# VinAIResearch/tise-toolbox

Hardware: AMD Instinct MI355X
Metric: images/sec through InceptionV3+FID on 30k 256x256 @1/2/4/8 GPU; |dFID| vs ref (higher is better)
Workload: dtype f32 (split 2xf16 operands, 3 f16 MFMAs/product, f32 accumulate)

## Files before the change

include/tise_hip.h:

```cpp
#ifndef TISE_HIP_H
#define TISE_HIP_H

#include <stddef.h>
#include <stdint.h>

#ifdef __cplusplus
extern "C" {
#endif

#define TISE_OK 0
#define TISE_ERR_INVALID_ARG (-1)
#define TISE_ERR_HIP (-2)
#define TISE_ERR_NO_DEVICE (-3)
#define TISE_ERR_UNSUPPORTED (-4)

const char* tise_status_string(int status);
int tise_last_hip_error(void);
int tise_version(void);
int tise_device_info(int* cu_count, int* gcn_arch_is_gfx950, size_t* total_mem);

int tise_host_register(void* host_ptr, size_t bytes);
int tise_host_unregister(void* host_ptr);
int tise_memcpy_h2d_async(void* dst_dev, const void* src_host, size_t bytes, void* stream);

// ... 105 lines not shown
                                            void* stream);
int tise_maxpool3s1p1_split_nhwc(const void* x_dev, int64_t x_ld, int x_off, int n, int h, int w,
                                 int C, void* out_dev, int64_t out_ld, int out_off, void* stream);

int tise_stem_conv3x3s2_split(const float* x_dev, int n, int h, int w, const float* w_dev, const float* bias_dev,
                              void* out_dev, void* stream);
int tise_stem_conv3x3s2_split_u8(const uint8_t* x_dev, const float* lut_dev, int n, int h, int w, const float* w_dev,
                                 const float* bias_dev, void* out_dev, void* stream);
int tise_stem_conv3x3s2_split_u8_mfma(const uint8_t* x_dev, const float* lut_dev, int n, int h, int w, const void* wsplit_dev,
                                      const float* scale_dev, const float* bias_dev, void* out_dev, void* stream);
int tise_split_mean_nhwc(const void* x_dev, int n, int hw, int C, float* out_dev, void* stream);
int tise_split_mean_both_nhwc(const void* x_dev, int n, int hw, int C, float* out_dev, void* out_split_dev, void* stream);

int tise_cosine_top1(const void* img_emb_dev, const void* txt_emb_dev, const int32_t* txt_index_dev, int64_t n, int c,
                     int d, int dtype, int normalize, float logit_scale, int32_t* top1_out_dev, float* p0_out_dev,
                     void* stream);

int tise_gemm_f16(const void* a_dev, int64_t lda, const void* w_dev, int64_t ldw, const void* bias_dev, const void* res_dev,
                  int64_t ldr, void* out_dev, int64_t ldo, int m, int n, int k, int act, void* stream);
int tise_layernorm_f16(const void* x_dev, int64_t ldx, const void* gamma_dev, const void* beta_dev, void* out_dev, int64_t ldo,
                       int64_t rows, int C, float eps, void* stream);
int tise_attention_f16(const void* qkv_dev, int batch, int seq, int heads, int head_dim, int causal, void* out_dev, void* stream);
int tise_patchify_f16(const void* img_dev, int batch, int res, int patch, void* out_dev, void* stream);
int tise_vit_tokens_f16(const void* patch_out_dev, const void* class_emb_dev, const void* pos_emb_dev, int batch, int n_patches,
                        int width, void* x_dev, void* stream);
int tise_text_tokens_f16(const int32_t* tokens_dev, const void* table_dev, const void* pos_emb_dev, int64_t rows, int seq, int width,
                         void* x_dev, void* stream);
int tise_gather_rows_f16(const void* x_dev, const int64_t* index_dev, int64_t n, int width, void* out_dev, void* stream);

typedef struct {
    int c0, c1;
    void* dst;
    long long ld;
    int off;
    int mode;
} tise_conv_seg;

typedef struct {
    const void* x;
    const void* w;
    long long w_plane;
    const float* scale;
    const float* bias;
    int N, H, W, Cin, KH, KW, SH, SW, PH, PW, OH, OW;
    int Cout, K, Kpad;
    long long M;
    int nseg;
    tise_conv_seg seg[4];
    int out_hp, out_wp, out_y0, out_x0;
} tise_conv_args;

int tise_conv_split_f16(const tise_conv_args* args, int tn, void* stream);

int tise_split_overflow_check(int* flag_host, void* stream);

int tise_gemm_f64(const double* a_dev, int64_t sam, int64_t sak, const double* b_dev, int64_t sbk,
                  int64_t sbn, double* c_dev, int64_t ldc, int m, int n, int k, void* stream);

#ifdef __cplusplus
}
#endif
#endif
```

tise_toolbox_amd/_lib.py:

```python
import ctypes
import os
from ctypes import POINTER, c_char_p, c_double, c_float, c_int, c_int64, c_size_t, c_uint8, c_void_p

_HERE = os.path.dirname(os.path.abspath(__file__))
LIB_PATH = os.environ.get("TISE_LIB_PATH") or os.path.join(_HERE, "libtise_hip.so")


class TiseLibraryError(RuntimeError):
    pass


class TiseStatusError(RuntimeError):
    def __init__(self, fn, status, detail):
        super().__init__(f"{fn} failed: {detail} (status {status})")
        self.status = status


TISE_OK = 0
TISE_ERR_INVALID_ARG = -1
TISE_ERR_HIP = -2
TISE_ERR_NO_DEVICE = -3
TISE_ERR_UNSUPPORTED = -4
TISE_FRECHET_OUT_DOUBLES = 8
TISE_FLAG_NONFINITE = 1
# ... 41 lines not shown
    "tise_mmd_poly3_workspace_bytes": (c_int, [POINTER(c_int64), POINTER(c_int64), c_int, POINTER(c_size_t)]),
    "tise_mmd_poly3_grouped": (c_int, [c_void_p, c_int64, c_int64, c_void_p, c_int64, POINTER(c_int64), c_void_p, c_int64, c_int64,
                                        c_void_p, c_int64, POINTER(c_int64), c_int, c_int, c_void_p, c_void_p, c_size_t, c_void_p]),
    "tise_mmd_rbf_workspace_bytes": (c_int, [POINTER(c_int64), POINTER(c_int64), c_int, POINTER(c_size_t)]),
    "tise_mmd_rbf_grouped": (c_int, [c_void_p, c_int64, c_int64, c_void_p, c_int64, POINTER(c_int64), c_void_p, c_int64, c_int64,
                                      c_void_p, c_int64, POINTER(c_int64), c_int, c_int, c_double, c_void_p, c_void_p, c_size_t,
                                      c_void_p]),
    "tise_knn_workspace_bytes": (c_int, [c_int64, c_int, c_int, POINTER(c_size_t)]),
    "tise_knn_radius2": (c_int, [c_void_p, c_int64, c_int64, c_int, c_int, c_int, c_void_p, c_void_p, c_size_t, c_void_p]),
    "tise_prdc_counts": (c_int, [c_void_p, c_int64, c_int64, c_void_p, c_void_p, c_int64, c_int64, c_void_p, c_int, c_int, c_void_p,
                                  c_void_p, c_void_p, c_void_p, c_size_t, c_void_p]),
    "tise_frechet_create": (c_int, [c_int, POINTER(c_void_p)]),
    "tise_frechet_destroy": (c_int, [c_void_p]),
    "tise_frechet_distance": (c_int, [c_void_p, c_void_p, c_void_p, c_void_p, c_void_p, c_double, c_void_p, c_void_p]),
    "tise_frechet_prefactor": (c_int, [c_void_p, c_void_p, c_void_p]),
    "tise_frechet_distance_prefactored": (c_int, [c_void_p, c_void_p, c_void_p, c_void_p, c_void_p, c_void_p, c_void_p]),
    "tise_frechet_prefactor_ms": (c_int, [c_void_p, POINTER(c_double)]),
    "tise_frechet_set_profiling": (c_int, [c_void_p, c_int]),
    "tise_frechet_phase_ms": (c_int, [c_void_p, POINTER(c_double), POINTER(c_int)]),
    "tise_eigvalsh": (c_int, [c_void_p, c_void_p, c_int, c_void_p, c_void_p]),
    "tise_pivoted_cholesky": (c_int, [c_void_p, c_void_p, c_void_p, POINTER(c_int), c_void_p]),
    "tise_frechet_factor": (c_int, [c_void_p, c_void_p, POINTER(c_int), POINTER(c_int), c_void_p]),
    "tise_is_update": (c_int, [c_void_p, c_int64, c_int64, c_int, c_double, c_int, c_int64, c_int64, c_int, c_int,
                                c_void_p, c_void_p, c_void_p]),
    "tise_is_finalize": (c_int, [c_void_p, c_int, c_int64, c_int, c_int, c_void_p, c_void_p]),
    "tise_calib_workspace_bytes": (c_int, [c_int64, c_int, c_int, POINTER(c_size_t)]),
    "tise_calib_eval": (c_int, [c_void_p, c_int64, c_int64, c_int, c_int, c_void_p, c_double, c_void_p, c_int, c_void_p,
                                 c_void_p, c_size_t, c_void_p]),
    "tise_bias_relu_nhwc": (c_int, [c_void_p, c_int64, c_int, c_int64, c_int, c_void_p, c_void_p, c_int64, c_int, c_void_p]),
    "tise_avgpool3_bias_relu_nhwc": (c_int, [c_void_p, c_int64, c_int, c_int, c_int, c_int, c_int, c_void_p, c_void_p,
                                              c_int64, c_int, c_void_p]),
    "tise_maxpool3s2_nhwc": (c_int, [c_void_p, c_int64, c_int, c_int, c_int, c_int, c_int, c_void_p, c_void_p, c_int64,
                                      c_int, c_void_p]),
    "tise_avgpool3_bias_relu_split_nhwc": (c_int, [c_void_p, c_int64, c_int, c_int, c_int, c_int, c_int, c_void_p,
                                                    c_void_p, c_int64, c_int, c_void_p]),
    "tise_maxpool3s2_split_nhwc": (c_int, [c_void_p, c_int64, c_int, c_int, c_int, c_int, c_int, c_void_p,
                                            c_int64, c_int, c_void_p]),
    "tise_avgpool3_excl_bias_relu_nhwc": (c_int, [c_void_p, c_int64, c_int, c_int, c_int, c_int, c_int, c_void_p, c_void_p,
                                                   c_int64, c_int, c_void_p]),
    "tise_maxpool3s1p1_nhwc": (c_int, [c_void_p, c_int64, c_int, c_int, c_int, c_int, c_int, c_void_p, c_int64, c_int,
                                        c_void_p]),
    "tise_avgpool3_excl_bias_relu_split_nhwc": (c_int, [c_void_p, c_int64, c_int, c_int, c_int, c_int, c_int, c_void_p,
                                                         c_void_p, c_int64, c_int, c_void_p]),
    "tise_maxpool3s1p1_split_nhwc": (c_int, [c_void_p, c_int64, c_int, c_int, c_int, c_int, c_int, c_void_p,
                                              c_int64, c_int, c_void_p]),
    "tise_stem_conv3x3s2_split": (c_int, [c_void_p, c_int, c_int, c_int, c_void_p, c_void_p, c_void_p, c_void_p]),
    "tise_stem_conv3x3s2_split_u8": (c_int, [c_void_p, c_void_p, c_int, c_int, c_int, c_void_p, c_void_p, c_void_p,
                                              c_void_p]),
    "tise_stem_conv3x3s2_split_u8_mfma": (c_int, [c_void_p, c_void_p, c_int, c_int, c_int, c_void_p, c_void_p, c_void_p,
                                                   c_void_p, c_void_p]),
    "tise_split_mean_nhwc": (c_int, [c_void_p, c_int, c_int, c_int, c_void_p, c_void_p]),
    "tise_split_mean_both_nhwc": (c_int, [c_void_p, c_int, c_int, c_int, c_void_p, c_void_p, c_void_p]),
    "tise_conv_split_f16": (c_int, [c_void_p, c_int, c_void_p]),
    "tise_split_overflow_check": (c_int, [POINTER(c_int), c_void_p]),
    "tise_gemm_f64": (c_int, [c_void_p, c_int64, c_int64, c_void_p, c_int64, c_int64, c_void_p, c_int64,
                               c_int, c_int, c_int, c_void_p]),
}

_lib = None


def load():
    global _lib
    if _lib is not None:
        return _lib
    if not os.path.exists(LIB_PATH):
        raise TiseLibraryError(
            f"{LIB_PATH} not found: build it with `python -m tise_toolbox_amd.build` "
            "(hipcc --offload-arch=gfx950).  There is no CPU fallback.")
    try:
        lib = ctypes.CDLL(LIB_PATH)
    except OSError as e:
        raise TiseLibraryError(f"cannot load {LIB_PATH}: {e}") from e
    for name, (res, args) in SIGNATURES.items():
        try:
            fn = getattr(lib, name)
        except AttributeError as e:
            raise TiseLibraryError(f"{LIB_PATH} does not export {name}") from e
        fn.restype = res
        fn.argtypes = args
    _lib = lib
    return lib


def check(fn_name, status):
    if status != TISE_OK:
        lib = load()
        detail = lib.tise_status_string(status).decode()
        if status == TISE_ERR_HIP:
            detail += f" (hipError_t {lib.tise_last_hip_error()})"
        raise TiseStatusError(fn_name, status, detail)


def call(fn_name, *args):
    lib = load()
    status = getattr(lib, fn_name)(*args)
    check(fn_name, status)
```

tise_toolbox_amd/csrc/conv_split.hip:

```cpp
#include <hip/hip_fp16.h>
#include "common.h"
#include "conv_epilogue.h"

typedef _Float16 half8_t __attribute__((ext_vector_type(8)));
typedef float float16_t __attribute__((ext_vector_type(16)));
typedef float float4_t __attribute__((ext_vector_type(4)));
typedef unsigned int u32x4_t __attribute__((ext_vector_type(4)));

#define CS_BM 128
#define CS_BK 32

typedef tise_conv_seg ConvSeg;
typedef tise_conv_args ConvArgs;

__device__ u32x4_t g_conv_zero_page[4];

typedef __attribute__((address_space(3))) void* lds_ptr_t;

template <int TN>
__global__ __launch_bounds__(256, 2) void conv_split_glds_kernel(const ConvArgs p) {
    constexpr int BN = 32 * TN;
    constexpr int A_PLANE = CS_BM * 64, B_PLANE = BN * 64;
    constexpr int STAGE = 2 * A_PLANE + 2 * B_PLANE;
    constexpr int T_BYTES = CS_BM * (BN * 2 + 16);
// ... 62 lines not shown
        if (a_c >= p.Cin) { a_c -= p.Cin; if (++a_kw == p.KW) { a_kw = 0; ++a_kh; } }                      \
        if (a_c >= p.Cin) { a_c -= p.Cin; if (++a_kw == p.KW) { a_kw = 0; ++a_kh; } }                      \
    }

    conv_epi::Acc16 acc_main[1][TN], acc_corr[1][TN];
#pragma unroll
    for (int t = 0; t < TN; ++t) { conv_epi::acc_zero(acc_main[0][t]); conv_epi::acc_zero(acc_corr[0][t]); }
    conv_epi::float4_t sc_pre = {0.f, 0.f, 0.f, 0.f}, bs_pre = {0.f, 0.f, 0.f, 0.f};
    if (tid < BN / 4) {
        sc_pre = *reinterpret_cast<const conv_epi::float4_t*>(p.scale + n0 + 4 * tid);
        bs_pre = *reinterpret_cast<const conv_epi::float4_t*>(p.bias + n0 + 4 * tid);
    }

    const int nsteps = p.Kpad / CS_BK;
    const int frow = (lane & 15) * 64;
    const int choff = (((lane >> 4)) ^ (((lane & 15) >> 2) & 3)) * 16;
    CG_ISSUE(0, lds)
    for (int step = 0; step < nsteps; ++step) {
        unsigned char* cur = lds + (step & 1) * STAGE;
        asm volatile("s_waitcnt vmcnt(0)" ::: "memory");
        __syncthreads();
        if (step + 1 < nsteps) CG_ISSUE(step + 1, lds + ((step + 1) & 1) * STAGE)
        half8_t a_[2][2];
#pragma unroll
        for (int pi = 0; pi < 2; ++pi) {
            const unsigned char* ap = cur + (wave * 32 + pi * 16) * 64 + frow + choff;
            a_[pi][0] = *reinterpret_cast<const half8_t*>(ap);
            a_[pi][1] = *reinterpret_cast<const half8_t*>(ap + A_PLANE);
        }
#pragma unroll
        for (int g = 0; g < 2 * TN; ++g) {
            const unsigned char* bp = cur + 2 * A_PLANE + g * 16 * 64 + frow + choff;
            const half8_t b_hi = *reinterpret_cast<const half8_t*>(bp);
            const half8_t b_lo = *reinterpret_cast<const half8_t*>(bp + B_PLANE);
#pragma unroll
            for (int pi = 0; pi < 2; ++pi) {
                float4_t& cm = acc_main[0][g >> 1].v[g & 1][pi];
                float4_t& cc = acc_corr[0][g >> 1].v[g & 1][pi];
                cm = __builtin_amdgcn_mfma_f32_16x16x32_f16(b_hi, a_[pi][0], cm, 0, 0, 0);
                cc = __builtin_amdgcn_mfma_f32_16x16x32_f16(b_lo, a_[pi][0], cc, 0, 0, 0);
                cc = __builtin_amdgcn_mfma_f32_16x16x32_f16(b_hi, a_[pi][1], cc, 0, 0, 0);
            }
        }
    }
    __syncthreads();
    constexpr int ETW = TN > 1 ? 2 : 1;
    constexpr int EPI0 = 4 * conv_epi::Staging<ETW>::BYTES;
    static_assert(EPI0 + conv_epi::EpiArea<BN>::BYTES <= LDS_BYTES, "epilogue staging must fit the operand LDS");
    conv_epi::prepare<BN>(p, lds + EPI0, n0, sc_pre, bs_pre);
    __syncthreads();
    conv_epi::store_tiles_desc<TN, ETW>(p, acc_main, acc_corr, lds + wave * conv_epi::Staging<ETW>::BYTES, lds + EPI0, m0 + wave * 32);
}

template <int TN, bool DBG = false, bool CBT = false>
__global__ __launch_bounds__(256, 2) void conv_split_fast_kernel(const ConvArgs p) {
    constexpr int BN = 32 * TN;
    constexpr int A_BYTES = CS_BM * 128, B_BYTES = BN * 128;
    constexpr int STAGE = A_BYTES + B_BYTES;
    constexpr int T_BYTES = CS_BM * (BN * 2 + 16);
    constexpr int LDS_BYTES = (2 * STAGE > T_BYTES) ? 2 * STAGE : T_BYTES;
    __shared__ __attribute__((aligned(1024))) unsigned char lds[LDS_BYTES];

    const int tid = threadIdx.x, lane = tid & 63;
    const int wave = __builtin_amdgcn_readfirstlane(tid >> 6);
    const unsigned tiles_n = (unsigned)(p.Cout + BN - 1) / BN;
    const unsigned nwg = gridDim.x;
    unsigned bid = blockIdx.x;
    {
        const unsigned q = nwg >> 3, r = nwg & 7, xcd = bid & 7, idx = bid >> 3;
        bid = ((xcd < r) ? xcd * (q + 1) : r * (q + 1) + (xcd - r) * q) + idx;
    }
    const unsigned tile_m = bid / tiles_n;
    const int tile_n = (int)(bid - tile_m * tiles_n);
    const long long m0 = (long long)tile_m * CS_BM;
    const int n0 = tile_n * BN;

    const unsigned char* zp = reinterpret_cast<const unsigned char*>(g_conv_zero_page);
    const int pix_bytes = p.Cin * 4;
    const unsigned char* pbase[4];
    int ihw[4];
    {
        const unsigned ohw = (unsigned)(p.OH * p.OW), M32 = (unsigned)p.M;
        const unsigned pix0 = tile_m * CS_BM + wave * 32 + (lane >> 3);
        const unsigned pp = pix0 < M32 ? pix0 : 0u;
        unsigned n = pp / ohw;
        const unsigned rem = pp - n * ohw;
        unsigned oh = rem / (unsigned)p.OW, ow = rem - oh * (unsigned)p.OW;
#pragma unroll
        for (int jj = 0; jj < 4; ++jj) {
            const int ih0 = (int)oh * p.SH - p.PH, iw0 = (int)ow * p.SW - p.PW;
            const bool rok = pix0 + 8 * jj < M32;
            ihw[jj] = rok ? ((ih0 + 0x4000) << 16) | (iw0 + 0x4000) : 0;
            pbase[jj] = reinterpret_cast<const unsigned char*>(p.x) +
                        (((long long)n * p.H + ih0) * p.W + iw0) * pix_bytes;
            ow += 8;
            while (ow >= (unsigned)p.OW) { ow -= (unsigned)p.OW; if (++oh == (unsigned)p.OH) { oh = 0; ++n; } }
        }
    }
    const unsigned char* wbase = reinterpret_cast<const unsigned char*>(p.w) + (long long)n0 * p.Kpad * 4;
    unsigned pb[TN];
    int pb_off[TN];
#pragma unroll
    for (int i = 0; i < TN; ++i) {
        const int q = wave * TN + i;
        const int r = q * 8 + (lane >> 3);
        const int c = (lane & 7) ^ tise_lds_swz(r);
        pb[i] = (unsigned)r * (unsigned)p.Kpad * 4u + c * 16;
        pb_off[i] = A_BYTES + q * 1024;
    }
    const unsigned char* pa[4];
    int pa_inc[4];
    int kh = 0, kw = 0, cblk = 0, istep = 0;
    const int ncblk = p.Cin / CS_BK, ntaps = p.KH * p.KW;
    const int nA = ntaps * ncblk;
    const int nB = (p.Cin & 16) ? (ntaps + 1) / 2 : 0;
    const int cl0 = (lane & 7) ^ ((lane >> 4) << 1), cl1 = cl0;
#define CF_TAP_ONE(JJ, KH_, KW_, CHB_, VALID_)                                                            \
    {                                                                                                     \
        const int ih = (ihw[JJ] >> 16) - 0x4000 + (KH_), iw = (ihw[JJ] & 0xffff) - 0x4000 + (KW_);         \
        const bool ok = (VALID_) && ih >= 0 && ih < p.H && iw >= 0 && iw < p.W;                            \
        const unsigned char* src = pbase[JJ] + ((KH_) * p.W + (KW_)) * pix_bytes + (CHB_);                 \
        pa[JJ] = ok ? src : zp;                                                                            \
        pa_inc[JJ] = ok ? 128 : 0;                                                                         \
    }
#define CF_TAP()                                                                                          \
    _Pragma("unroll") for (int jj = 0; jj < 4; ++jj) CF_TAP_ONE(jj, kh, kw, ((jj & 1) ? cl1 : cl0) * 16, kh < p.KH)
#define CF_TAP_B(J)                                                                                       \
    _Pragma("unroll") for (int par = 0; par < 2; ++par) {                                                  \
        const int c_ = par ? cl1 : cl0;                                                                    \
        const int tl = 2 * (J) + ((c_ >> 1) & 1);                                                          \
        const int lkh = tl / p.KW, lkw = tl - lkh * p.KW;                                                  \
        const int chb = ncblk * 128 + (c_ >> 2) * 32 + (c_ & 1) * 16;                                      \
        CF_TAP_ONE(par, lkh, lkw, chb, tl < ntaps)                                                         \
        CF_TAP_ONE(par + 2, lkh, lkw, chb, tl < ntaps)                                                     \
    }
#define CF_ISSUE(STAGEOFF)                                                                                \
    {                                                                                                     \
        _Pragma("unroll") for (int jj = 0; jj < 4; ++jj) {                                                 \
                                                     \
            const unsigned char* sa = pa[jj];                                                              \
             \
            if (!(DBG && (p.nseg & 0x1000)) || istep % 7 == 0)                                             \
                __builtin_amdgcn_global_load_lds(sa, (lds_ptr_t)(lds + (STAGEOFF) + (4 * wave + jj) * 1024), 16, 0, 0); \
            pa[jj] = sa + pa_inc[jj];                                                                      \
        }                                                                                                  \
        _Pragma("unroll") for (int i = 0; i < TN; ++i) {                                                   \
            const unsigned char* sw_ = wbase + pb[i];                                                      \
            unsigned char* dw_ = lds + (STAGEOFF) + pb_off[i];                                             \
            __builtin_amdgcn_global_load_lds(sw_, (lds_ptr_t)dw_, 16, 0, 0);                               \
            pb[i] += 128;                                              \
        }                                                                                                  \
        ++istep;                                              \
        if constexpr (CBT) {                                  \
            int delta = pix_bytes - 128;                      \
            if (++kw == p.KW) {                                                                            \
                kw = 0;                                                                                    \
                delta = (p.W - p.KW + 1) * pix_bytes - 128;          \
                if (++kh == p.KH) { kh = 0; delta = -((p.KH - 1) * p.W + (p.KW - 1)) * pix_bytes; }    \
            }                                                                                              \
            _Pragma("unroll") for (int jj = 0; jj < 4; ++jj) pa[jj] += (long long)(pa_inc[jj] ? delta : 0); \
        } else if (istep >= nA) {                                                        \
            if (istep < nA + nB) CF_TAP_B(istep - nA)                                                      \
        } else if (++cblk == ncblk) {                                                 \
            cblk = 0;                                                                                      \
            if (++kw == p.KW) { kw = 0; ++kh; }                                                            \
            CF_TAP()                                                                                       \
        }                                                                                                  \
    }

    constexpr bool W22 = TN == 4;
    constexpr int NPH = W22 ? 4 : 2;
    constexpr int NCH = W22 ? TN : 2 * TN;
    constexpr int RG = NPH / 2, TNW = NCH / 2;
    const int wm = W22 ? (wave & 1) : wave, wn = W22 ? (wave >> 1) : 0;
    conv_epi::Acc16 acc_main[RG][1][TNW], acc_corr[RG][1][TNW];
#pragma unroll
    for (int r = 0; r < RG; ++r)
#pragma unroll
        for (int t = 0; t < TNW; ++t) { conv_epi::acc_zero(acc_main[r][0][t]); conv_epi::acc_zero(acc_corr[r][0][t]); }
    constexpr bool PRE = TN < 5;
    conv_epi::float4_t sc_pre = {0.f, 0.f, 0.f, 0.f}, bs_pre = {0.f, 0.f, 0.f, 0.f};
    if (PRE && tid < BN / 4) {
        sc_pre = *reinterpret_cast<const conv_epi::float4_t*>(p.scale + n0 + 4 * tid);
        bs_pre = *reinterpret_cast<const conv_epi::float4_t*>(p.bias + n0 + 4 * tid);
    }

    const int nsteps = nA + nB;
    const int f16o = (lane & 15) * 128 + (((lane >> 4) ^ tise_lds_swz(lane & 15)) << 4);
    const unsigned char* fa = lds + wm * NPH * 2048;
    const int fbw = A_BYTES + wn * NCH * 2048;
    half8_t h_a[NPH][2], h_b[2];

#define CF_HEAD(STAGEOFF)                                                                                 \
    {                                                                                                     \
        _Pragma("unroll") for (int pi = 0; pi < NPH; ++pi) {                                               \
            h_a[pi][0] = *reinterpret_cast<const half8_t*>(fa + (STAGEOFF) + pi * 2048 + f16o);            \
            h_a[pi][1] = *reinterpret_cast<const half8_t*>(fa + (STAGEOFF) + pi * 2048 + (f16o ^ 64));     \
        }                                                                                                  \
        h_b[0] = *reinterpret_cast<const half8_t*>(lds + (STAGEOFF) + fbw + f16o);                         \
        h_b[1] = *reinterpret_cast<const half8_t*>(lds + (STAGEOFF) + fbw + (f16o ^ 64));                  \
        __builtin_amdgcn_sched_barrier(0);                                                                 \
    }
#define CF_COMPUTE(STAGEOFF)                                                                              \
    {                                                                                                     \
        __builtin_amdgcn_sched_barrier(0);                                                                 \
        half8_t fb_[NCH][2];                                                                               \
        _Pragma("unroll") for (int g = 0; g < NCH; ++g) {                                                  \
            if (g == 0) { fb_[0][0] = h_b[0]; fb_[0][1] = h_b[1]; }                                        \
            else {                                                                                         \
                const unsigned char* bb = lds + (STAGEOFF) + fbw + g * 2048;                               \
                fb_[g][0] = *reinterpret_cast<const half8_t*>(bb + f16o);                                  \
                fb_[g][1] = *reinterpret_cast<const half8_t*>(bb + (f16o ^ 64));                           \
            }                                                                                              \
        }                                                                                                  \
        _Pragma("unroll") for (int g = 0; g < NCH; ++g)                                                    \
            _Pragma("unroll") for (int pi = 0; pi < NPH; ++pi) {                                           \
                           \
                float4_t& cm = acc_main[pi >> 1][0][g >> 1].v[g & 1][pi & 1];                              \
                float4_t& cc = acc_corr[pi >> 1][0][g >> 1].v[g & 1][pi & 1];                              \
                cc = __builtin_amdgcn_mfma_f32_16x16x32_f16(fb_[g][1], h_a[pi][0], cc, 0, 0, 0);           \
                cm = __builtin_amdgcn_mfma_f32_16x16x32_f16(fb_[g][0], h_a[pi][0], cm, 0, 0, 0);           \
                cc = __builtin_amdgcn_mfma_f32_16x16x32_f16(fb_[g][0], h_a[pi][1], cc, 0, 0, 0);           \
            }                                                                                              \
        _Pragma("unroll") for (int g = 0; g < NCH; ++g) {                                                  \
            if (g + 1 < NCH) __builtin_amdgcn_sched_group_barrier(0x100, 2, 0);              \
            __builtin_amdgcn_sched_group_barrier(0x008, 3 * NPH, 0);                        \
        }                                                                                                  \
    }

    const bool ab_dma = !(p.nseg & 0x100), ab_mma = !(p.nseg & 0x200);
    const bool dbg = DBG && (p.nseg & 0x800) && blockIdx.x == 0;
    int* dbuf = reinterpret_cast<int*>(p.seg[3].dst);
#define CF_STAMP(STEP, K)                                                                                  \
    if (DBG && dbg && lane == 0 && (STEP) < 96) dbuf[wave * 512 + (STEP) * 5 + (K)] = (int)__builtin_readcyclecounter();
    if (dbg && lane == 0) dbuf[wave * 512 + 480] = (int)(__builtin_amdgcn_s_memrealtime());
#define CF_BAR() { __builtin_amdgcn_sched_barrier(0); __builtin_amdgcn_s_barrier(); __builtin_amdgcn_sched_barrier(0); }
    int step = 0;
    CF_TAP()
    CF_ISSUE(0)
    for (; step + 1 < nsteps; step += 2) {
        CF_STAMP(step, 0)
        asm volatile("s_waitcnt vmcnt(0)" ::: "memory");
        CF_STAMP(step, 1)
        __syncthreads();
        CF_STAMP(step, 2)
        CF_HEAD(0)
        if (ab_dma) CF_ISSUE(STAGE)
        CF_STAMP(step, 3)
        if (ab_mma) CF_COMPUTE(0)
        CF_STAMP(step, 4)
        CF_STAMP(step + 1, 0)
        asm volatile("s_waitcnt vmcnt(0)" ::: "memory");
        CF_STAMP(step + 1, 1)
        __syncthreads();
        CF_STAMP(step + 1, 2)
        CF_HEAD(STAGE)
        if (step + 2 < nsteps && ab_dma) CF_ISSUE(0)
        CF_STAMP(step + 1, 3)
        if (ab_mma) CF_COMPUTE(STAGE)
        CF_STAMP(step + 1, 4)
    }
    if (dbg && lane == 0) dbuf[wave * 512 + 481] = (int)(__builtin_amdgcn_s_memrealtime());
    if (step < nsteps) {
        asm volatile("s_waitcnt vmcnt(0)" ::: "memory");
        __syncthreads();
        CF_HEAD(0)
        CF_COMPUTE(0)
    }
    __syncthreads();
    if ((p.nseg & 0x400) && p.M > 0) return;
    constexpr int ETW = TN > 1 ? 2 : 1;
    constexpr int EPI0 = 4 * conv_epi::Staging<ETW>::BYTES;
    static_assert(EPI0 + conv_epi::EpiArea<BN>::BYTES <= LDS_BYTES, "epilogue staging must fit the operand LDS");
    if (!PRE && tid < BN / 4) {
        sc_pre = *reinterpret_cast<const conv_epi::float4_t*>(p.scale + n0 + 4 * tid);
        bs_pre = *reinterpret_cast<const conv_epi::float4_t*>(p.bias + n0 + 4 * tid);
    }
    conv_epi::prepare<BN>(p, lds + EPI0, n0, sc_pre, bs_pre, tid);
    __syncthreads();
#pragma unroll
    for (int r = 0; r < RG; ++r)
        conv_epi::store_tiles_desc<TNW, ETW, false, BN>(p, acc_main[r], acc_corr[r], lds + wave * conv_epi::Staging<ETW>::BYTES, lds + EPI0,
                                                        m0 + wm * NPH * 16 + r * 32, wn * NCH * 2);
}


template <int TN, int NP, bool POOLH = false>
__global__ __launch_bounds__(256, 2) void conv_split_rowwin_kernel(const ConvArgs p, const unsigned inv_wp) {
    constexpr int BN = 32 * TN;
    constexpr int MSTEP = POOLH ? 126 : CS_BM;
    constexpr int A_BYTES = NP * 4 * 1024;
    constexpr int B_BYTES = BN * 128;
    constexpr int B0 = 2 * A_BYTES;
    constexpr int LDS_BYTES = 2 * A_BYTES + 2 * B_BYTES;
    extern __shared__ __attribute__((aligned(1024))) unsigned char lds[];

    const int tid = threadIdx.x, lane = tid & 63;
    const int wave = __builtin_amdgcn_readfirstlane(tid >> 6);
    const unsigned tiles_n = (unsigned)(p.Cout + BN - 1) / BN;
    const unsigned nwg = gridDim.x;
    unsigned bid = blockIdx.x;
    {
        const unsigned q = nwg >> 3, r = nwg & 7, xcd = bid & 7, idx = bid >> 3;
        bid = ((xcd < r) ? xcd * (q + 1) : r * (q + 1) + (xcd - r) * q) + idx;
    }
    const unsigned tile_m = bid / tiles_n;
    const int tile_n = (int)(bid - tile_m * tiles_n);
    const long long m0 = (long long)tile_m * MSTEP;
    const int n0 = tile_n * BN;
    const unsigned char* zp = reinterpret_cast<const unsigned char*>(g_conv_zero_page);
    const int pix_bytes = p.Cin * 4;
    const int Wp = p.OW + p.KW - 1;
    const unsigned row0 = (unsigned)(tile_m * MSTEP) / (unsigned)p.OW;
    const int x0 = (int)(tile_m * MSTEP - row0 * (unsigned)p.OW);
    const unsigned img0 = row0 / (unsigned)p.OH;
    const int oy0 = (int)(row0 - img0 * (unsigned)p.OH);
    const unsigned nrows_out = (unsigned)p.N * (unsigned)p.OH;

    const unsigned char* pbase[NP];
    int oyp[NP];
    const int cch = (lane & 7) ^ ((lane >> 4) << 1);
    const int full_off = cch * 16;
    const int tail_off = (cch >> 2) * 32 + (cch & 1) * 16;
    const bool tail_has = (cch & 3) < 2;
#pragma unroll
    for (int t = 0; t < NP; ++t) {
        const int q = wave + 4 * t;
        const int rho = 8 * q + (lane >> 3);
        const unsigned u = (unsigned)(rho + x0);
        const unsigned j = (u * inv_wp) >> 16;
        const int xin = (int)(u - j * (unsigned)Wp) - p.PW;
        unsigned n = img0;
        int oy = oy0 + (int)j;
        while (oy >= p.OH) { oy -= p.OH; ++n; }
        const bool okx = xin >= 0 && xin < p.W && row0 + j < nrows_out;
        oyp[t] = okx ? oy - p.PH + 0x4000 : 0;
// ... 371 lines not shown
        __syncthreads();
        if (step + 1 < nsteps) PI_B_ISSUE(((step + 1) & 1) * B_BYTES)
        half8_t a_[2][2];
#pragma unroll
        for (int pi = 0; pi < 2; ++pi) {
            a_[pi][0] = *reinterpret_cast<const half8_t*>(fa + pi * 2048 + f16o);
            a_[pi][1] = *reinterpret_cast<const half8_t*>(fa + pi * 2048 + (f16o ^ 64));
        }
#pragma unroll
        for (int g = 0; g < 2 * TNW; ++g) {
            const unsigned char* bb = lds + A_BYTES + bcur + (wn * 2 * TNW + g) * 2048;
            const half8_t b_hi = *reinterpret_cast<const half8_t*>(bb + f16o);
            const half8_t b_lo = *reinterpret_cast<const half8_t*>(bb + (f16o ^ 64));
#pragma unroll
            for (int pi = 0; pi < 2; ++pi) {
                float4_t& cm = acc_main[0][g >> 1].v[g & 1][pi];
                float4_t& cc = acc_corr[0][g >> 1].v[g & 1][pi];
                cc = __builtin_amdgcn_mfma_f32_16x16x32_f16(b_lo, a_[pi][0], cc, 0, 0, 0);
                cm = __builtin_amdgcn_mfma_f32_16x16x32_f16(b_hi, a_[pi][0], cm, 0, 0, 0);
                cc = __builtin_amdgcn_mfma_f32_16x16x32_f16(b_hi, a_[pi][1], cc, 0, 0, 0);
            }
        }
    }
#undef PI_B_ISSUE
    __syncthreads();
    conv_epi::prepare<BN>(p, lds + EPI0, n0, sc_pre, bs_pre);
    __syncthreads();
    conv_epi::store_tiles_desc<TNW, ETW, false, BN>(p, acc_main, acc_corr, lds + wave * conv_epi::Staging<ETW>::BYTES, lds + EPI0,
                                                    m0 + wm * 32, wn * TNW * 4);
}

static int launch_poolin(const ConvArgs* a, int tn, hipStream_t st, bool vt = false) {
    if (a->KH != 1 || a->KW != 1 || a->PH != 0 || a->PW != 0 || a->Cin % 32 != 0 || a->Kpad != a->Cin || a->H < 3 || a->W < (vt ? 1 : 3) ||
        a->OH != (a->H - 3) / 2 + 1 || a->OW != (vt ? a->W : (a->W - 3) / 2 + 1) || a->M != (long long)a->N * a->OH * a->OW || a->M >= 0x7fffff00LL ||
        (long long)a->W * a->Cin * 4 * 3 >= 0x7fffffffLL)
        return TISE_ERR_INVALID_ARG;
    (void)tn;
    const int tnw = a->Cout <= 128 ? 2 : 4;
    const int bn = 64 * tnw;
    const long long tiles = ((a->M + 63) / 64) * ((a->Cout + bn - 1) / bn);
    if (tiles > 0x7fffffffLL) return TISE_ERR_UNSUPPORTED;
    const dim3 grid((unsigned)tiles), block(256);
    if (vt) {
        if (tnw == 2) hipLaunchKernelGGL((conv_poolin_kernel<2, true>), grid, block, 0, st, *a);
        else hipLaunchKernelGGL((conv_poolin_kernel<4, true>), grid, block, 0, st, *a);
    } else if (tnw == 2) hipLaunchKernelGGL(conv_poolin_kernel<2>, grid, block, 0, st, *a);
    else hipLaunchKernelGGL(conv_poolin_kernel<4>, grid, block, 0, st, *a);
    TISE_LAUNCH_CHECK();
    return TISE_OK;
}

int tise_conv_pipe_launch(const tise_conv_args* a, int cfg, void* stream);

extern "C" int tise_conv_split_f16(const ConvArgs* args, int tn, void* stream) {
    if (!args || !args->x || !args->w || !args->scale || !args->bias || (args->nseg & 0xff) < 1 || (args->nseg & 0xff) > 4 ||
        args->Cin % 16 != 0 || args->Cin < 32 || (args->Kpad % CS_BK != 0 && !(tn & 512)) || args->M <= 0)
        return TISE_ERR_INVALID_ARG;
    for (int i = 0; i < (args->nseg & 0xff); ++i) {
        const tise_conv_seg& g = args->seg[i];
        const int al = g.mode == 0 ? 8 : 4;
        if (!g.dst || g.c0 % 8 != 0 || g.c1 <= g.c0 || g.off % al != 0 || g.ld % (g.mode == 0 ? 16 : 4) != 0 ||
            (g.mode == 0 && g.off + (g.c1 - g.c0) > g.ld) ||
            (reinterpret_cast<uintptr_t>(g.dst) & 15) != 0 || (i > 0 && g.c0 != args->seg[i - 1].c1) || (g.mode != 0 && g.mode != 1))
            return TISE_ERR_INVALID_ARG;
        const bool last = i == (args->nseg & 0xff) - 1;
        const int c_end = ((last ? args->Cout : g.c1) + 7) / 8 * 8;
        if (g.mode == 1 && g.off + (c_end - g.c0) > g.ld) return TISE_ERR_INVALID_ARG;
    }
    if (args->seg[0].c0 != 0) return TISE_ERR_INVALID_ARG;
    if (tn & 512) return tise_conv_pipe_launch(args, (tn & 255) | (tn & 1024), stream);
    if (args->out_hp | args->out_wp | args->out_y0 | args->out_x0) return TISE_ERR_INVALID_ARG;
    if (tn & 256) return launch_poolin(args, tn & 15, (hipStream_t)stream, (tn & 2048) != 0);
    if (tn & 64) return launch_rowwin_any(args, tn & 15, (hipStream_t)stream, (tn & 2048) != 0);
    const bool glds = (tn & 16) != 0;
    const int fast_kpad = (args->KH * args->KW * (args->Cin / 32) + ((args->Cin & 16) ? (args->KH * args->KW + 1) / 2 : 0)) * 32;
    const bool fast = (tn & 128) != 0 && args->Cin % 16 == 0 && args->Kpad == fast_kpad && args->M < 0x7fffff00LL &&
                      args->H < 0x3f00 && args->W < 0x3f00 && args->PH < 0x100 && args->PW < 0x100;
    if ((tn & 128) && !fast) return TISE_ERR_UNSUPPORTED;
    const bool cbt = (tn & 4096) != 0;
    tn &= 15;
    const int bn = 32 * tn;
    const int bm = CS_BM;
    const long long tiles = ((args->M + bm - 1) / bm) * ((args->Cout + bn - 1) / bn);
    if (tiles > 0x7fffffffLL) return TISE_ERR_UNSUPPORTED;
    const dim3 grid((unsigned)tiles), block(256);
    hipStream_t st = (hipStream_t)stream;
    if (fast && (args->nseg & 0x800)) {
        switch (tn) {
            case 3: hipLaunchKernelGGL((conv_split_fast_kernel<3, true>), grid, block, 0, st, *args); break;
            case 4: hipLaunchKernelGGL((conv_split_fast_kernel<4, true>), grid, block, 0, st, *args); break;
            default: return TISE_ERR_INVALID_ARG;
        }
        TISE_LAUNCH_CHECK();
        return TISE_OK;
    }
    if (fast && cbt) {
        if (args->PH != 0 || args->PW != 0 || args->Cin % 32 != 0 || args->KH * args->KW < 2) return TISE_ERR_INVALID_ARG;
        switch (tn) {
            case 2: hipLaunchKernelGGL((conv_split_fast_kernel<2, false, true>), grid, block, 0, st, *args); break;
            case 3: hipLaunchKernelGGL((conv_split_fast_kernel<3, false, true>), grid, block, 0, st, *args); break;
            case 4: hipLaunchKernelGGL((conv_split_fast_kernel<4, false, true>), grid, block, 0, st, *args); break;
            case 5: hipLaunchKernelGGL((conv_split_fast_kernel<5, false, true>), grid, block, 0, st, *args); break;
            default: return TISE_ERR_INVALID_ARG;
        }
        TISE_LAUNCH_CHECK();
        return TISE_OK;
    }
    if (fast) {
        switch (tn) {
            case 1: hipLaunchKernelGGL(conv_split_fast_kernel<1>, grid, block, 0, st, *args); break;
            case 2: hipLaunchKernelGGL(conv_split_fast_kernel<2>, grid, block, 0, st, *args); break;
            case 3: hipLaunchKernelGGL(conv_split_fast_kernel<3>, grid, block, 0, st, *args); break;
            case 4: hipLaunchKernelGGL(conv_split_fast_kernel<4>, grid, block, 0, st, *args); break;
            case 5: hipLaunchKernelGGL(conv_split_fast_kernel<5>, grid, block, 0, st, *args); break;
            default: return TISE_ERR_INVALID_ARG;
        }
        TISE_LAUNCH_CHECK();
        return TISE_OK;
    }
    if (glds) {
        switch (tn) {
            case 1: hipLaunchKernelGGL(conv_split_glds_kernel<1>, grid, block, 0, st, *args); break;
            case 2: hipLaunchKernelGGL(conv_split_glds_kernel<2>, grid, block, 0, st, *args); break;
            case 3: hipLaunchKernelGGL(conv_split_glds_kernel<3>, grid, block, 0, st, *args); break;
            case 4: hipLaunchKernelGGL(conv_split_glds_kernel<4>, grid, block, 0, st, *args); break;
            case 5: hipLaunchKernelGGL(conv_split_glds_kernel<5>, grid, block, 0, st, *args); break;
            default: return TISE_ERR_INVALID_ARG;
        }
        TISE_LAUNCH_CHECK();
        return TISE_OK;
    }
    return TISE_ERR_INVALID_ARG;
}

TISE_DEFINE_SPLIT_FLAG_READER(tise_internal_split_flag_conv_split)
```

Baseline: 25890.

## Add paired-tile conv kernel sharing weight LDS and half-width last N tile

Refactors the fast split-f16 conv body into a device function and adds two variants. The first is a paired form: a 512-thread block runs two M tiles that share a triple-buffered weight stage in LDS, with staggered B prefetch and finer vmcnt waits. The second is a narrow form that runs the last N tile at half width when Cout leaves a small remainder. By default the pair rule returns false, but narrow is enabled whenever TN=4, there is no CBT, and the last tile is at most half width, so default runs use it to avoid wasted MFMA work on padded columns.

```diff
diff --git a/include/tise_hip.h b/include/tise_hip.h
--- a/include/tise_hip.h
+++ b/include/tise_hip.h
@@ -181,6 +181,8 @@
 
 int tise_conv_split_f16(const tise_conv_args* args, int tn, void* stream);
 
+int tise_conv_split_last_form(void);
+
 int tise_split_overflow_check(int* flag_host, void* stream);
 
 int tise_gemm_f64(const double* a_dev, int64_t sam, int64_t sak, const double* b_dev, int64_t sbk,
diff --git a/tise_toolbox_amd/_lib.py b/tise_toolbox_amd/_lib.py
--- a/tise_toolbox_amd/_lib.py
+++ b/tise_toolbox_amd/_lib.py
@@ -117,6 +117,7 @@
     "tise_split_mean_nhwc": (c_int, [c_void_p, c_int, c_int, c_int, c_void_p, c_void_p]),
     "tise_split_mean_both_nhwc": (c_int, [c_void_p, c_int, c_int, c_int, c_void_p, c_void_p, c_void_p]),
     "tise_conv_split_f16": (c_int, [c_void_p, c_int, c_void_p]),
+    "tise_conv_split_last_form": (c_int, []),
     "tise_split_overflow_check": (c_int, [POINTER(c_int), c_void_p]),
     "tise_gemm_f64": (c_int, [c_void_p, c_int64, c_int64, c_void_p, c_int64, c_int64, c_void_p, c_int64,
                                c_int, c_int, c_int, c_void_p]),
diff --git a/tise_toolbox_amd/csrc/conv_split.hip b/tise_toolbox_amd/csrc/conv_split.hip
--- a/tise_toolbox_amd/csrc/conv_split.hip
+++ b/tise_toolbox_amd/csrc/conv_split.hip
@@ -138,28 +138,35 @@
     conv_epi::store_tiles_desc<TN, ETW>(p, acc_main, acc_corr, lds + wave * conv_epi::Staging<ETW>::BYTES, lds + EPI0, m0 + wave * 32);
 }
 
-template <int TN, bool DBG = false, bool CBT = false>
-__global__ __launch_bounds__(256, 2) void conv_split_fast_kernel(const ConvArgs p) {
+template <int TN, bool PAIR>
+struct ConvFastLds {
+    static constexpr int BN = 32 * TN;
+    static constexpr int A_BYTES = CS_BM * 128, B_BYTES = BN * 128;
+    static constexpr int STAGE = A_BYTES + B_BYTES;
+    static constexpr int T_BYTES = CS_BM * (BN * 2 + 16);
+    static constexpr int SOLO_BYTES = (2 * STAGE > T_BYTES) ? 2 * STAGE : T_BYTES;
+    static constexpr int EPI_STRIDE = ((4 * conv_epi::Staging<(TN > 1 ? 2 : 1)>::BYTES + conv_epi::EpiArea<BN>::BYTES + 1023) / 1024) * 1024;
+    static constexpr int PAIR_OPER = 4 * A_BYTES + 3 * B_BYTES;
+    static constexpr int PAIR_BYTES = PAIR_OPER > 2 * EPI_STRIDE ? PAIR_OPER : 2 * EPI_STRIDE;
+    static constexpr int BYTES = PAIR ? PAIR_BYTES : SOLO_BYTES;
+};
+
+template <int TN, bool DBG, bool CBT, bool PAIR>
+__device__ __forceinline__ void conv_fast_tile(const ConvArgs& p, unsigned char* const lds_all, const unsigned tile_m, const int n0) {
+    static_assert(!PAIR || (TN % 2 == 0 && !DBG), "paired form: even tile widths (equal weight shares of the halves), no instrumentation");
     constexpr int BN = 32 * TN;
-    constexpr int A_BYTES = CS_BM * 128, B_BYTES = BN * 128;
-    constexpr int STAGE = A_BYTES + B_BYTES;
-    constexpr int T_BYTES = CS_BM * (BN * 2 + 16);
-    constexpr int LDS_BYTES = (2 * STAGE > T_BYTES) ? 2 * STAGE : T_BYTES;
-    __shared__ __attribute__((aligned(1024))) unsigned char lds[LDS_BYTES];
-
-    const int tid = threadIdx.x, lane = tid & 63;
+    constexpr int A_BYTES = ConvFastLds<TN, PAIR>::A_BYTES, B_BYTES = ConvFastLds<TN, PAIR>::B_BYTES;
+    constexpr int STAGE = ConvFastLds<TN, PAIR>::STAGE;
+    constexpr int LDS_BYTES = ConvFastLds<TN, PAIR>::BYTES;
+    constexpr int NB = PAIR ? TN / 2 : TN;
+
+    const int tid = PAIR ? (threadIdx.x & 255) : threadIdx.x, lane = tid & 63;
     const int wave = __builtin_amdgcn_readfirstlane(tid >> 6);
-    const unsigned tiles_n = (unsigned)(p.Cout + BN - 1) / BN;
-    const unsigned nwg = gridDim.x;
-    unsigned bid = blockIdx.x;
-    {
-        const unsigned q = nwg >> 3, r = nwg & 7, xcd = bid & 7, idx = bid >> 3;
-        bid = ((xcd < r) ? xcd * (q + 1) : r * (q + 1) + (xcd - r) * q) + idx;
-    }
-    const unsigned tile_m = bid / tiles_n;
-    const int tile_n = (int)(bid - tile_m * tiles_n);
+    const int half = PAIR ? __builtin_amdgcn_readfirstlane(threadIdx.x >> 8) : 0;
+    unsigned char* const lds = lds_all + (PAIR ? half * 2 * A_BYTES : 0);
+    unsigned char* const ldsb = PAIR ? lds_all + 4 * A_BYTES : lds_all + A_BYTES;
+    unsigned char* const lds_e = lds_all + (PAIR ? half * ConvFastLds<TN, PAIR>::EPI_STRIDE : 0);
     const long long m0 = (long long)tile_m * CS_BM;
-    const int n0 = tile_n * BN;
 
     const unsigned char* zp = reinterpret_cast<const unsigned char*>(g_conv_zero_page);
     const int pix_bytes = p.Cin * 4;
@@ -184,15 +191,15 @@
         }
     }
     const unsigned char* wbase = reinterpret_cast<const unsigned char*>(p.w) + (long long)n0 * p.Kpad * 4;
-    unsigned pb[TN];
-    int pb_off[TN];
-#pragma unroll
-    for (int i = 0; i < TN; ++i) {
-        const int q = wave * TN + i;
+    unsigned pb[NB];
+    int pb_off[NB];
+#pragma unroll
+    for (int i = 0; i < NB; ++i) {
+        const int q = (half * 4 + wave) * NB + i;
         const int r = q * 8 + (lane >> 3);
         const int c = (lane & 7) ^ tise_lds_swz(r);
         pb[i] = (unsigned)r * (unsigned)p.Kpad * 4u + c * 16;
-        pb_off[i] = A_BYTES + q * 1024;
+        pb_off[i] = q * 1024;
     }
     const unsigned char* pa[4];
     int pa_inc[4];
@@ -220,22 +227,25 @@
         CF_TAP_ONE(par, lkh, lkw, chb, tl < ntaps)                                                         \
         CF_TAP_ONE(par + 2, lkh, lkw, chb, tl < ntaps)                                                     \
     }
-#define CF_ISSUE(STAGEOFF)                                                                                \
-    {                                                                                                     \
+#define CF_ISSUE(STAGEOFF) { CF_ISSUE_A_DMA(STAGEOFF) CF_ISSUE_B(STAGEOFF) CF_ADVANCE() }
+#define CF_ISSUE_A(AOFF) { CF_ISSUE_A_DMA(AOFF) CF_ADVANCE() }
+#define CF_ISSUE_A_DMA(AOFF)                                                                              \
         _Pragma("unroll") for (int jj = 0; jj < 4; ++jj) {                                                 \
                                                      \
             const unsigned char* sa = pa[jj];                                                              \
              \
             if (!(DBG && (p.nseg & 0x1000)) || istep % 7 == 0)                                             \
-                __builtin_amdgcn_global_load_lds(sa, (lds_ptr_t)(lds + (STAGEOFF) + (4 * wave + jj) * 1024), 16, 0, 0); \
+                __builtin_amdgcn_global_load_lds(sa, (lds_ptr_t)(lds + (AOFF) + (4 * wave + jj) * 1024), 16, 0, 0); \
             pa[jj] = sa + pa_inc[jj];                                                                      \
-        }                                                                                                  \
-        _Pragma("unroll") for (int i = 0; i < TN; ++i) {                                                   \
+        }
+#define CF_ISSUE_B(BOFF)                                                                                  \
+        _Pragma("unroll") for (int i = 0; i < NB; ++i) {                                                   \
             const unsigned char* sw_ = wbase + pb[i];                                                      \
-            unsigned char* dw_ = lds + (STAGEOFF) + pb_off[i];                                             \
+            unsigned char* dw_ = ldsb + (BOFF) + pb_off[i];                                                \
             __builtin_amdgcn_global_load_lds(sw_, (lds_ptr_t)dw_, 16, 0, 0);                               \
             pb[i] += 128;                                              \
-        }                                                                                                  \
+        }
+#define CF_ADVANCE()                                                                                      \
         ++istep;                                              \
         if constexpr (CBT) {                                  \
             int delta = pix_bytes - 128;                      \
@@ -251,8 +261,7 @@
             cblk = 0;                                                                                      \
             if (++kw == p.KW) { kw = 0; ++kh; }                                                            \
             CF_TAP()                                                                                       \
-        }                                                                                                  \
-    }
+        }
 
     constexpr bool W22 = TN == 4;
     constexpr int NPH = W22 ? 4 : 2;
@@ -270,31 +279,33 @@
         sc_pre = *reinterpret_cast<const conv_epi::float4_t*>(p.scale + n0 + 4 * tid);
         bs_pre = *reinterpret_cast<const conv_epi::float4_t*>(p.bias + n0 + 4 * tid);
     }
+    if constexpr (PAIR) __builtin_amdgcn_sched_barrier(0);
 
     const int nsteps = nA + nB;
     const int f16o = (lane & 15) * 128 + (((lane >> 4) ^ tise_lds_swz(lane & 15)) << 4);
     const unsigned char* fa = lds + wm * NPH * 2048;
-    const int fbw = A_BYTES + wn * NCH * 2048;
+    const int fbw = wn * NCH * 2048;
     half8_t h_a[NPH][2], h_b[2];
 
-#define CF_HEAD(STAGEOFF)                                                                                 \
+#define CF_HEAD(STAGEOFF) CF_HEAD2(STAGEOFF, STAGEOFF)
+#define CF_HEAD2(AOFF, BOFF)                                                                              \
     {                                                                                                     \
         _Pragma("unroll") for (int pi = 0; pi < NPH; ++pi) {                                               \
-            h_a[pi][0] = *reinterpret_cast<const half8_t*>(fa + (STAGEOFF) + pi * 2048 + f16o);            \
-            h_a[pi][1] = *reinterpret_cast<const half8_t*>(fa + (STAGEOFF) + pi * 2048 + (f16o ^ 64));     \
+            h_a[pi][0] = *reinterpret_cast<const half8_t*>(fa + (AOFF) + pi * 2048 + f16o);                \
+            h_a[pi][1] = *reinterpret_cast<const half8_t*>(fa + (AOFF) + pi * 2048 + (f16o ^ 64));         \
         }                                                                                                  \
-        h_b[0] = *reinterpret_cast<const half8_t*>(lds + (STAGEOFF) + fbw + f16o);                         \
-        h_b[1] = *reinterpret_cast<const half8_t*>(lds + (STAGEOFF) + fbw + (f16o ^ 64));                  \
+        h_b[0] = *reinterpret_cast<const half8_t*>(ldsb + (BOFF) + fbw + f16o);                            \
+        h_b[1] = *reinterpret_cast<const half8_t*>(ldsb + (BOFF) + fbw + (f16o ^ 64));                     \
         __builtin_amdgcn_sched_barrier(0);                                                                 \
     }
-#define CF_COMPUTE(STAGEOFF)                                                                              \
+#define CF_COMPUTE(BOFF)                                                                                  \
     {                                                                                                     \
         __builtin_amdgcn_sched_barrier(0);                                                                 \
         half8_t fb_[NCH][2];                                                                               \
         _Pragma("unroll") for (int g = 0; g < NCH; ++g) {                                                  \
             if (g == 0) { fb_[0][0] = h_b[0]; fb_[0][1] = h_b[1]; }                                        \
             else {                                                                                         \
-                const unsigned char* bb = lds + (STAGEOFF) + fbw + g * 2048;                               \
+                const unsigned char* bb = ldsb + (BOFF) + fbw + g * 2048;                                  \
                 fb_[g][0] = *reinterpret_cast<const half8_t*>(bb + f16o);                                  \
                 fb_[g][1] = *reinterpret_cast<const half8_t*>(bb + (f16o ^ 64));                           \
             }                                                                                              \
@@ -322,52 +333,139 @@
     if (dbg && lane == 0) dbuf[wave * 512 + 480] = (int)(__builtin_amdgcn_s_memrealtime());
 #define CF_BAR() { __builtin_amdgcn_sched_barrier(0); __builtin_amdgcn_s_barrier(); __builtin_amdgcn_sched_barrier(0); }
     int step = 0;
-    CF_TAP()
-    CF_ISSUE(0)
-    for (; step + 1 < nsteps; step += 2) {
-        CF_STAMP(step, 0)
-        asm volatile("s_waitcnt vmcnt(0)" ::: "memory");
-        CF_STAMP(step, 1)
-        __syncthreads();
-        CF_STAMP(step, 2)
-        CF_HEAD(0)
-        if (ab_dma) CF_ISSUE(STAGE)
-        CF_STAMP(step, 3)
-        if (ab_mma) CF_COMPUTE(0)
-        CF_STAMP(step, 4)
-        CF_STAMP(step + 1, 0)
-        asm volatile("s_waitcnt vmcnt(0)" ::: "memory");
-        CF_STAMP(step + 1, 1)
-        __syncthreads();
-        CF_STAMP(step + 1, 2)
-        CF_HEAD(STAGE)
-        if (step + 2 < nsteps && ab_dma) CF_ISSUE(0)
-        CF_STAMP(step + 1, 3)
-        if (ab_mma) CF_COMPUTE(STAGE)
-        CF_STAMP(step + 1, 4)
-    }
-    if (dbg && lane == 0) dbuf[wave * 512 + 481] = (int)(__builtin_amdgcn_s_memrealtime());
-    if (step < nsteps) {
-        asm volatile("s_waitcnt vmcnt(0)" ::: "memory");
-        __syncthreads();
-        CF_HEAD(0)
-        CF_COMPUTE(0)
+    if constexpr (PAIR) {
+        constexpr int PA = 4;
+        int b_iss = 0, b_cmp = 0;
+#define CF_BNEXT(V) V = ((V) == 2 * B_BYTES) ? 0 : (V) + B_BYTES;
+#define CF_ISSUE_BH() { CF_ISSUE_B(b_iss) CF_BNEXT(b_iss) }
+#define CF_WAIT_OLDER(MORE_A, MORE_B)                                                                     \
+        {                                                                                                  \
+            if ((MORE_A) && (MORE_B)) asm volatile("s_waitcnt vmcnt(%0)" ::"n"(PA + NB) : "memory");       \
+            else if (MORE_A) asm volatile("s_waitcnt vmcnt(%0)" ::"n"(PA) : "memory");                     \
+            else asm volatile("s_waitcnt vmcnt(0)" ::: "memory");                                          \
+        }
+#define CF_PAIR_STEP(S, ACUR, ANEXT)                                                                      \
+        {                                                                                                  \
+            CF_BAR()                                                                                       \
+            const bool more_a = (S) + 1 < nsteps, more_b = (S) + lead < nsteps;                            \
+            if (more_a) CF_ISSUE_A(ANEXT)                                                                  \
+            if (more_b) CF_ISSUE_BH()                                                                      \
+            CF_WAIT_OLDER(more_a, more_b)                                                                  \
+            CF_BAR()                                                                                       \
+            CF_HEAD2(ACUR, b_cmp)                                                                          \
+            CF_COMPUTE(b_cmp)                                                                              \
+            CF_BNEXT(b_cmp)                                                                                \
+        }
+        const int lead = 1 + half;
+        CF_TAP()
+        if (half == 0) {
+            CF_ISSUE_A(0)
+            CF_ISSUE_BH()
+        } else {
+            CF_ISSUE_BH()
+            if (nsteps > 1) CF_ISSUE_BH()
+            CF_ISSUE_A(0)
+            if (nsteps > 1) asm volatile("s_waitcnt vmcnt(%0)" ::"n"(PA + NB) : "memory");
+            else asm volatile("s_waitcnt vmcnt(%0)" ::"n"(PA) : "memory");
+            CF_BAR()
+        }
+        for (; step + 1 < nsteps; step += 2) {
+            CF_PAIR_STEP(step, 0, A_BYTES)
+            CF_PAIR_STEP(step + 1, A_BYTES, 0)
+        }
+        if (step < nsteps) CF_PAIR_STEP(step, 0, A_BYTES)
+        if (half == 0) CF_BAR()
+#undef CF_PAIR_STEP
+#undef CF_WAIT_OLDER
+#undef CF_ISSUE_BH
+#undef CF_BNEXT
+    } else {
+        CF_TAP()
+        CF_ISSUE(0)
+        for (; step + 1 < nsteps; step += 2) {
+            CF_STAMP(step, 0)
+            asm volatile("s_waitcnt vmcnt(0)" ::: "memory");
+            CF_STAMP(step, 1)
+            __syncthreads();
+            CF_STAMP(step, 2)
+            CF_HEAD(0)
+            if (ab_dma) CF_ISSUE(STAGE)
+            CF_STAMP(step, 3)
+            if (ab_mma) CF_COMPUTE(0)
+            CF_STAMP(step, 4)
+            CF_STAMP(step + 1, 0)
+            asm volatile("s_waitcnt vmcnt(0)" ::: "memory");
+            CF_STAMP(step + 1, 1)
+            __syncthreads();
+            CF_STAMP(step + 1, 2)
+            CF_HEAD(STAGE)
+            if (step + 2 < nsteps && ab_dma) CF_ISSUE(0)
+            CF_STAMP(step + 1, 3)
+            if (ab_mma) CF_COMPUTE(STAGE)
+            CF_STAMP(step + 1, 4)
+        }
+        if (dbg && lane == 0) dbuf[wave * 512 + 481] = (int)(__builtin_amdgcn_s_memrealtime());
+        if (step < nsteps) {
+            asm volatile("s_waitcnt vmcnt(0)" ::: "memory");
+            __syncthreads();
+            CF_HEAD(0)
+            CF_COMPUTE(0)
+        }
     }
     __syncthreads();
     if ((p.nseg & 0x400) && p.M > 0) return;
     constexpr int ETW = TN > 1 ? 2 : 1;
     constexpr int EPI0 = 4 * conv_epi::Staging<ETW>::BYTES;
-    static_assert(EPI0 + conv_epi::EpiArea<BN>::BYTES <= LDS_BYTES, "epilogue staging must fit the operand LDS");
+    static_assert(EPI0 + conv_epi::EpiArea<BN>::BYTES <= (PAIR ? ConvFastLds<TN, PAIR>::EPI_STRIDE : LDS_BYTES), "epilogue staging must fit the operand LDS");
     if (!PRE && tid < BN / 4) {
         sc_pre = *reinterpret_cast<const conv_epi::float4_t*>(p.scale + n0 + 4 * tid);
         bs_pre = *reinterpret_cast<const conv_epi::float4_t*>(p.bias + n0 + 4 * tid);
     }
-    conv_epi::prepare<BN>(p, lds + EPI0, n0, sc_pre, bs_pre, tid);
+    conv_epi::prepare<BN>(p, lds_e + EPI0, n0, sc_pre, bs_pre, tid);
     __syncthreads();
 #pragma unroll
     for (int r = 0; r < RG; ++r)
-        conv_epi::store_tiles_desc<TNW, ETW, false, BN>(p, acc_main[r], acc_corr[r], lds + wave * conv_epi::Staging<ETW>::BYTES, lds + EPI0,
+        conv_epi::store_tiles_desc<TNW, ETW, false, BN>(p, acc_main[r], acc_corr[r], lds_e + wave * conv_epi::Staging<ETW>::BYTES, lds_e + EPI0,
                                                         m0 + wm * NPH * 16 + r * 32, wn * NCH * 2);
+#undef CF_TAP_ONE
+#undef CF_TAP
+#undef CF_TAP_B
+#undef CF_ISSUE
+#undef CF_ISSUE_A
+#undef CF_ISSUE_A_DMA
+#undef CF_ISSUE_B
+#undef CF_ADVANCE
+#undef CF_HEAD
+#undef CF_HEAD2
+#undef CF_COMPUTE
+#undef CF_STAMP
+#undef CF_BAR
+}
+
+template <int TN, bool DBG = false, bool CBT = false, bool PAIR = false, bool NARROW = false>
+__global__ __launch_bounds__(PAIR ? 512 : 256, PAIR ? 1 : 2) void conv_split_fast_kernel(const ConvArgs p) {
+    static_assert(!NARROW || TN == 4, "the half-width last tile is built for TN = 4");
+    constexpr int BN = 32 * TN;
+    __shared__ __attribute__((aligned(1024))) unsigned char lds[ConvFastLds<TN, PAIR>::BYTES];
+    const unsigned tiles_n = (unsigned)(p.Cout + BN - 1) / BN;
+    const unsigned nwg = gridDim.x;
+    unsigned bid = blockIdx.x;
+    {
+        const unsigned q = nwg >> 3, r = nwg & 7, xcd = bid & 7, idx = bid >> 3;
+        bid = ((xcd < r) ? xcd * (q + 1) : r * (q + 1) + (xcd - r) * q) + idx;
+    }
+    unsigned tile_m = bid / tiles_n;
+    const int tile_n = (int)(bid - tile_m * tiles_n);
+    if (PAIR) tile_m = 2 * tile_m + (unsigned)__builtin_amdgcn_readfirstlane(threadIdx.x >> 8);
+    const int n0 = tile_n * BN;
+    if constexpr (NARROW) {
+        if (p.Cout - n0 <= BN / 2) {
+            static_assert(ConvFastLds<TN / 2, PAIR>::BYTES <= ConvFastLds<TN, PAIR>::BYTES, "the narrow body runs in the wide body's LDS");
+            conv_fast_tile<TN / 2, DBG, CBT, PAIR>(p, lds, tile_m, n0);
+            return;
+        }
+    }
+    conv_fast_tile<TN, DBG, CBT, PAIR>(p, lds, tile_m, n0);
 }
 
 
@@ -845,6 +943,14 @@
 
 int tise_conv_pipe_launch(const tise_conv_args* a, int cfg, void* stream);
 
+static std::atomic<int> g_conv_last_form{0};
+extern "C" int tise_conv_split_last_form(void) { return g_conv_last_form.load(std::memory_order_relaxed); }
+static bool conv_rule_narrow(const ConvArgs* a, long long tiles_n) { (void)a; return tiles_n > 1; }
+static bool conv_rule_pair(const ConvArgs* a, int tn, bool cbt, long long tiles_m, long long tiles_n) {
+    (void)a; (void)tn; (void)cbt; (void)tiles_m; (void)tiles_n;
+    return false;
+}
+
 extern "C" int tise_conv_split_f16(const ConvArgs* args, int tn, void* stream) {
     if (!args || !args->x || !args->w || !args->scale || !args->bias || (args->nseg & 0xff) < 1 || (args->nseg & 0xff) > 4 ||
         args->Cin % 16 != 0 || args->Cin < 32 || (args->Kpad % CS_BK != 0 && !(tn & 512)) || args->M <= 0)
@@ -887,8 +993,30 @@
         TISE_LAUNCH_CHECK();
         return TISE_OK;
     }
+    if (fast && cbt && (args->PH != 0 || args->PW != 0 || args->Cin % 32 != 0 || args->KH * args->KW < 2)) return TISE_ERR_INVALID_ARG;
+    if (fast) {
+        const char* pe = getenv("TISE_CONV_PAIRED");
+        const int pmode = pe ? atoi(pe) : -1;
+        const long long tiles_m = (args->M + bm - 1) / bm, tiles_n = (args->Cout + bn - 1) / bn;
+        const int last_n = args->Cout - (int)(tiles_n - 1) * bn;
+        const bool can_narrow = tn == 4 && !cbt && last_n <= bn / 2;
+        const bool can_pair = (tn == 2 || tn == 4) && !(args->nseg & ~0xff);
+        const bool narrow = can_narrow && (pmode < 0 ? conv_rule_narrow(args, tiles_n) : (pmode & 2) != 0);
+        const bool pair = can_pair && (pmode < 0 ? conv_rule_pair(args, tn, cbt, tiles_m, tiles_n) : (pmode & 1) != 0);
+        g_conv_last_form.store((pair ? 1 : 0) | (narrow ? 2 : 0), std::memory_order_relaxed);
+        if (pair || narrow) {
+            const dim3 pgrid((unsigned)(pair ? ((tiles_m + 1) / 2) * tiles_n : tiles)), pblock(pair ? 512 : 256);
+            if (tn == 2 && !cbt) hipLaunchKernelGGL((conv_split_fast_kernel<2, false, false, true>), pgrid, pblock, 0, st, *args);
+            else if (tn == 2) hipLaunchKernelGGL((conv_split_fast_kernel<2, false, true, true>), pgrid, pblock, 0, st, *args);
+            else if (cbt) hipLaunchKernelGGL((conv_split_fast_kernel<4, false, true, true>), pgrid, pblock, 0, st, *args);
+            else if (pair && narrow) hipLaunchKernelGGL((conv_split_fast_kernel<4, false, false, true, true>), pgrid, pblock, 0, st, *args);
+            else if (pair) hipLaunchKernelGGL((conv_split_fast_kernel<4, false, false, true>), pgrid, pblock, 0, st, *args);
+            else hipLaunchKernelGGL((conv_split_fast_kernel<4, false, false, false, true>), pgrid, pblock, 0, st, *args);
+            TISE_LAUNCH_CHECK();
+            return TISE_OK;
+        }
+    }
     if (fast && cbt) {
-        if (args->PH != 0 || args->PW != 0 || args->Cin % 32 != 0 || args->KH * args->KW < 2) return TISE_ERR_INVALID_ARG;
         switch (tn) {
             case 2: hipLaunchKernelGGL((conv_split_fast_kernel<2, false, true>), grid, block, 0, st, *args); break;
             case 3: hipLaunchKernelGGL((conv_split_fast_kernel<3, false, true>), grid, block, 0, st, *args); break;
```

Result: no change. 25900, median of 2 (+0.1%).
